# JeffreyXiang/ivid

Measured on NVIDIA H100. Metric: 128x128 RGBD multiview samples/sec, higher is better.
Workload: dtype fp16 tensor-core operands, fp32 accumulate / residual stream / GroupNorm / softmax / sampler

## Files before the change

### include/ivid_b200.h

```cpp
#ifndef IVID_B200_H_
#define IVID_B200_H_

#include <stdint.h>

#ifdef __cplusplus
extern "C" {
#endif

#define IVID_OK 0
#define IVID_ERR_INVALID_ARGUMENT 1
#define IVID_ERR_NOT_IMPLEMENTED 2
#define IVID_ERR_CUDA 3
#define IVID_ERR_STATE 4

typedef struct ivid_unet ivid_unet_t;
typedef struct ivid_sampler ivid_sampler_t;

const char* ivid_last_error(void);
int ivid_version(void);
int ivid_device_info(int device, int* sm_count, int* cc_major, int* cc_minor);


int ivid_unet_create(const char* cfg_json, ivid_unet_t** out);
int ivid_unet_destroy(ivid_unet_t* h);

int ivid_unet_num_params(const ivid_unet_t* h, int* count);
int ivid_unet_param_info(const ivid_unet_t* h, int index, const char** name, int64_t shape[4], int* ndim,
                         int* is_buffer);
int ivid_unet_set_param(ivid_unet_t* h, const char* name, const float* host_data, const int64_t* shape, int ndim);
int ivid_unet_finalize(ivid_unet_t* h, int device);
int ivid_unet_set_precision(ivid_unet_t* h, int precision);
int ivid_fp8_e4m3_quantize(const float* in, uint8_t* out, uint64_t count);
int ivid_fp8_weight_exponent(const float* w, uint64_t count, int* e_out);
int ivid_unet_weight_arena(const ivid_unet_t* h, void** dev_ptr, uint64_t* bytes);

int ivid_unet_forward(ivid_unet_t* h, const float* x_dev, int Nx, const int64_t* t_dev, const int64_t* classes_dev,
                      float* eps_dev, int N, void* stream);

int ivid_conv_tile(int H, int W, int* tw, int* th, int* tn, int* fused_stats);

int ivid_unet_debug_tap(ivid_unet_t* h, int N, const char* layer, float* host_out, uint64_t capacity, int* C, int* H, int* W);

int ivid_unet_profile_begin(ivid_unet_t* h);
int ivid_unet_profile_end(ivid_unet_t* h, char* json_out, int capacity);

typedef struct {
  int kind;
  const float* y_dev;
  const float* mask_dev;
  const float* mask_rgb_dev;
  const float* noise_dev;
  uint64_t seed;
  uint32_t stream_id;
  int sr_scale;
} ivid_cond_t;
int ivid_unet_forward_cond(ivid_unet_t* h, const float* x_dev, int Nx, const ivid_cond_t* cond, const int64_t* t_dev,
                           const int64_t* classes_dev, float* eps_dev, int N, void* stream);

int ivid_unet_forward_hw(ivid_unet_t* h, const float* x_dev, int Nx, int H, int W, const ivid_cond_t* cond,
                         const int64_t* t_dev, const int64_t* classes_dev, float* eps_dev, int N, void* stream);

int ivid_unet_forward_reuse(ivid_unet_t* h, const float* x_dev, int Nx, int H, int W, const ivid_cond_t* cond,
                            const int64_t* t_dev, const int64_t* classes_dev, float* eps_dev, int N, int cache_branch,
                            void* stream);


int ivid_sampler_create(const double* betas, int timesteps, ivid_sampler_t** out);
int ivid_sampler_destroy(ivid_sampler_t* s);
int ivid_sampler_table(const ivid_sampler_t* s, int which, double* out, int count);

typedef struct {
  int kind;
  int use_cfg;
  float strength;
  int clip_denoised;
  float eta;
  const int64_t* classes_dev;
  ivid_cond_t cond;
  const float* replace_rgb_dev;
  const float* replace_rgb_mask_dev;
  double replace_rgb_weight;
  const float* replace_depth_dev;
  const float* replace_depth_mask_dev;
  double replace_depth_weight;
  const float* constrain_depth_dev;
  double constrain_depth_weight;
  const float* step_noise_dev;
  uint64_t seed;
  int height, width;
  int order;
  const float* prev_x0_dev;
  int t_last;
// ... 108 lines not shown
```

### ivid_b200/_lib.py

```python
from __future__ import annotations

import ctypes
import os
from ctypes import POINTER, Structure, byref, c_char_p, c_double, c_float, c_int, c_int64, c_uint32, c_uint64, c_void_p

_HERE = os.path.dirname(os.path.abspath(__file__))
LIB_PATH = os.path.join(_HERE, "libivid_b200.so")

IVID_OK = 0
IVID_ERR_INVALID_ARGUMENT = 1
IVID_ERR_NOT_IMPLEMENTED = 2
IVID_ERR_CUDA = 3
IVID_ERR_STATE = 4


class CondT(Structure):
    _fields_ = [
        ("kind", c_int),
        ("y_dev", c_void_p),
        ("mask_dev", c_void_p),
        ("mask_rgb_dev", c_void_p),
        ("noise_dev", c_void_p),
        ("seed", c_uint64),
        ("stream_id", c_uint32),
# ... 39 lines not shown


class OpConvT(Structure):
    _fields_ = [
        ("act0_dev", c_void_p), ("C0", c_int), ("ksize", c_int), ("w0_host", c_void_p), ("b0_host", c_void_p),
        ("e4m3", c_int), ("e_out", POINTER(c_int)),
        ("act1_dev", c_void_p), ("C1", c_int), ("act2_dev", c_void_p), ("C2", c_int), ("wskip_host", c_void_p),
        ("bskip_host", c_void_p),
        ("residual_dev", c_void_p), ("residual_up", c_int),
        ("N", c_int), ("H", c_int), ("W", c_int), ("Cout", c_int),
        ("out_dev", c_void_p), ("out_mode", c_int), ("out16_dev", c_void_p), ("stats_dev", c_void_p),
    ]


class OpGnT(Structure):
    _fields_ = [
        ("x0_dev", c_void_p), ("C0", c_int), ("x1_dev", c_void_p), ("C1", c_int), ("x_fp16", c_int),
        ("stats0_dev", c_void_p), ("stats1_dev", c_void_p),
        ("N", c_int), ("H", c_int), ("W", c_int), ("groups", c_int), ("eps", c_float),
        ("gamma_host", c_void_p), ("beta_host", c_void_p),
        ("film_dev", c_void_p), ("film_ld", c_int), ("film_off", c_int), ("film_add", c_int),
        ("silu", c_int), ("mode", c_int),
        ("out_dev", c_void_p), ("out_e4m3", c_int), ("out_lo_dev", c_void_p), ("out_raw16_dev", c_void_p),
        ("out_raw32_dev", c_void_p),
    ]


class WarpParamsT(Structure):
    _fields_ = [("fov_deg", c_double), ("near", c_double), ("far", c_double), ("atol", c_double), ("rtol", c_double),
                ("erode_rgb", c_int), ("padding", c_double)]


SIGNATURES = {
    "ivid_last_error": (c_char_p, []),
    "ivid_version": (c_int, []),
    "ivid_device_info": (c_int, [c_int, POINTER(c_int), POINTER(c_int), POINTER(c_int)]),
    "ivid_unet_create": (c_int, [c_char_p, POINTER(c_void_p)]),
    "ivid_unet_destroy": (c_int, [c_void_p]),
    "ivid_unet_num_params": (c_int, [c_void_p, POINTER(c_int)]),
    "ivid_unet_param_info": (c_int, [c_void_p, c_int, POINTER(c_char_p), POINTER(c_int64), POINTER(c_int), POINTER(c_int)]),
    "ivid_unet_set_param": (c_int, [c_void_p, c_char_p, c_void_p, POINTER(c_int64), c_int]),
    "ivid_unet_finalize": (c_int, [c_void_p, c_int]),
    "ivid_unet_weight_arena": (c_int, [c_void_p, POINTER(c_void_p), POINTER(c_uint64)]),
    "ivid_unet_set_precision": (c_int, [c_void_p, c_int]),
    "ivid_fp8_e4m3_quantize": (c_int, [c_void_p, c_void_p, c_uint64]),
    "ivid_fp8_weight_exponent": (c_int, [c_void_p, c_uint64, POINTER(c_int)]),
    "ivid_unet_forward": (c_int, [c_void_p, c_void_p, c_int, c_void_p, c_void_p, c_void_p, c_int, c_void_p]),
    "ivid_unet_forward_cond": (c_int, [c_void_p, c_void_p, c_int, POINTER(CondT), c_void_p, c_void_p, c_void_p, c_int, c_void_p]),
    "ivid_unet_forward_hw": (c_int, [c_void_p, c_void_p, c_int, c_int, c_int, POINTER(CondT), c_void_p, c_void_p, c_void_p, c_int,
                                     c_void_p]),
    "ivid_unet_forward_reuse": (c_int, [c_void_p, c_void_p, c_int, c_int, c_int, POINTER(CondT), c_void_p, c_void_p, c_void_p,
                                        c_int, c_int, c_void_p]),
    "ivid_conv_tile": (c_int, [c_int, c_int, POINTER(c_int), POINTER(c_int), POINTER(c_int), POINTER(c_int)]),
    "ivid_unet_debug_tap": (c_int, [c_void_p, c_int, c_char_p, c_void_p, c_uint64, POINTER(c_int), POINTER(c_int), POINTER(c_int)]),
    "ivid_unet_profile_begin": (c_int, [c_void_p]),
    "ivid_unet_profile_end": (c_int, [c_void_p, c_char_p, c_int]),
    "ivid_sampler_create": (c_int, [POINTER(c_double), c_int, POINTER(c_void_p)]),
    "ivid_sampler_destroy": (c_int, [c_void_p]),
    "ivid_sampler_table": (c_int, [c_void_p, c_int, POINTER(c_double), c_int]),
    "ivid_sampler_step": (c_int, [c_void_p, c_void_p, c_void_p, c_void_p, c_void_p, c_int, c_int, c_int, POINTER(StepArgsT), c_void_p]),
    "ivid_sampler_step_dev": (c_int, [c_void_p, c_void_p, c_void_p, c_void_p, c_void_p, c_int, c_void_p, c_void_p, POINTER(StepArgsT), c_void_p]),
    "ivid_cfg_mix": (c_int, [c_void_p, c_float, c_void_p, c_uint64, c_void_p]),
    "ivid_op_dynamic_threshold": (c_int, [c_void_p, c_int, c_int, c_double, c_double, c_void_p, c_void_p, c_void_p]),
    "ivid_sampler_run": (c_int, [c_void_p, c_void_p, c_void_p, c_int, c_int, POINTER(StepArgsT), c_void_p, c_void_p, c_void_p, c_void_p, c_void_p]),
    "ivid_op_conv2d": (c_int, [c_void_p, c_int, c_int, c_int, c_int, c_void_p, c_void_p, c_int, c_int, c_void_p, c_int,
                               c_void_p, c_void_p, c_void_p, c_void_p, c_int, c_void_p]),
    "ivid_op_group_norm": (c_int, [c_void_p, c_int, c_void_p, c_int, c_int, c_int, c_int, c_int, c_float, c_void_p, c_void_p,
                                   c_void_p, c_int, c_int, c_void_p, c_void_p]),
    "ivid_op_conv2d_e4m3": (c_int, [c_void_p, c_int, c_int, c_int, c_int, c_void_p, c_void_p, c_int, c_int, c_void_p, c_int,
                                    c_void_p, c_void_p, c_void_p, c_void_p, c_int, POINTER(c_int), c_void_p]),
    "ivid_op_group_norm_e4m3": (c_int, [c_void_p, c_int, c_void_p, c_int, c_int, c_int, c_int, c_int, c_float, c_void_p,
                                        c_void_p, c_void_p, c_int, c_int, c_void_p, c_void_p]),
    "ivid_op_conv2d_ex": (c_int, [POINTER(OpConvT), c_void_p]),
    "ivid_op_group_norm_apply": (c_int, [POINTER(OpGnT), c_void_p]),
    "ivid_op_attention": (c_int, [c_void_p, c_int, c_int, c_int, c_void_p, c_void_p]),
    "ivid_op_attention_heads": (c_int, [c_void_p, c_int, c_int, c_int, c_int, c_void_p, c_void_p]),
    "ivid_warp_create": (c_int, [c_int, c_int, c_int, c_int, c_double, c_double, c_int, POINTER(c_void_p)]),
    "ivid_warp_destroy": (c_int, [c_void_p]),
    "ivid_warp_reset": (c_int, [c_void_p]),
    "ivid_warp_num_views": (c_int, [c_void_p, POINTER(c_int)]),
    "ivid_warp_add_view": (c_int, [c_void_p, c_void_p, c_void_p, c_int, POINTER(WarpParamsT), c_void_p]),
    "ivid_warp_mesh_from_depth": (c_int, [c_void_p, c_void_p, c_void_p, POINTER(WarpParamsT), c_void_p, c_void_p, c_void_p]),
    "ivid_warp_set_mesh": (c_int, [c_void_p, c_int, c_int, c_void_p, c_void_p, c_void_p, c_void_p]),
    "ivid_warp_get_mesh": (c_int, [c_void_p, c_int, c_int, c_void_p, c_void_p, c_void_p]),
    "ivid_warp_render": (c_int, [c_void_p, c_void_p, c_int, c_double, c_void_p, c_void_p, c_void_p, c_void_p, c_void_p]),
    "ivid_warp_aggregate": (c_int, [c_void_p, c_void_p, c_int, POINTER(WarpParamsT), c_void_p, c_void_p]),
    "ivid_warp_resolve_frame": (c_int, [c_void_p, c_double, c_double, c_void_p, c_void_p, c_void_p, c_void_p]),
    "ivid_warp_render_simple": (c_int, [c_void_p, c_void_p, c_int, c_void_p, c_int, c_void_p, c_void_p, c_double, c_void_p, c_void_p, c_void_p, c_void_p]),
    "ivid_warp_forward_backward": (c_int, [c_void_p, c_void_p, c_void_p, c_void_p, c_void_p, c_int, POINTER(WarpParamsT), c_void_p, c_void_p]),
    "ivid_warp_postfilter": (c_int, [c_void_p, c_void_p, c_void_p, c_void_p, c_void_p, POINTER(WarpParamsT), c_void_p, c_void_p]),
}

_lib = None


def lib() -> ctypes.CDLL:
    global _lib
    if _lib is None:
        if not os.path.exists(LIB_PATH):
            raise ImportError(
                f"{LIB_PATH} not found: build it with `python -m ivid_b200.build` (ivid_b200 has no CPU fallback)")
        l = ctypes.CDLL(LIB_PATH)
        for name, (res, args) in SIGNATURES.items():
            try:
                fn = getattr(l, name)
            except AttributeError:
# ... 33 lines not shown
```

### ivid_b200/csrc/api.cu

```cuda
#include <algorithm>
#include <cmath>
#include <cstring>
#include <memory>
#include <string>
#include <vector>

#include "../../include/ivid_b200.h"
#include "ops.h"
#include "sampler.h"
#include "unet.h"

using namespace ivid;

struct ivid_unet { std::unique_ptr<Unet> impl; };
struct ivid_sampler { std::unique_ptr<Sampler> impl; };

static thread_local std::string g_last_error;
namespace ivid { void set_last_error(const std::string& msg) { g_last_error = msg; } }

template <class F>
static int guarded(F&& f) {
  try {
    f();
    return IVID_OK;
// ... 84 lines not shown
  return guarded([&] {
    IVID_REQUIRE(count == 0 || w != nullptr, "w must not be NULL");
    IVID_NOT_NULL(e_out);
    float mx = 0.f;
    for (uint64_t i = 0; i < count; ++i) mx = std::max(mx, std::fabs(w[i]));
    *e_out = fp8_weight_exponent(mx);
  });
}
int ivid_unet_weight_arena(const ivid_unet_t* h, void** dev_ptr, uint64_t* bytes) {
  return guarded([&] {
    IVID_NOT_NULL(h);
    if (!h->impl->finalized()) throw Error(kErrState, "weight arena requested before finalize");
    if (dev_ptr) *dev_ptr = h->impl->arena();
    if (bytes) *bytes = h->impl->arena_bytes();
  });
}
int ivid_unet_forward_hw(ivid_unet_t* h, const float* x_dev, int Nx, int H, int W, const ivid_cond_t* cond,
                         const int64_t* t_dev, const int64_t* classes_dev, float* eps_dev, int N, void* stream) {
  return guarded([&] {
    IVID_NOT_NULL(h); IVID_NOT_NULL(x_dev); IVID_NOT_NULL(t_dev); IVID_NOT_NULL(eps_dev);
    h->impl->forward(x_dev, Nx, H, W, cond, t_dev, classes_dev, eps_dev, N, static_cast<cudaStream_t>(stream));
  });
}
int ivid_unet_forward_reuse(ivid_unet_t* h, const float* x_dev, int Nx, int H, int W, const ivid_cond_t* cond,
                            const int64_t* t_dev, const int64_t* classes_dev, float* eps_dev, int N, int cache_branch,
                            void* stream) {
  return guarded([&] {
    IVID_NOT_NULL(h); IVID_NOT_NULL(x_dev); IVID_NOT_NULL(t_dev); IVID_NOT_NULL(eps_dev);
    IVID_REQUIRE(cache_branch >= 0, "cache_branch must be in [0, num_res_blocks]");
    h->impl->forward(x_dev, Nx, H, W, cond, t_dev, classes_dev, eps_dev, N, static_cast<cudaStream_t>(stream), nullptr,
                     cache_branch);
  });
}
int ivid_unet_forward(ivid_unet_t* h, const float* x_dev, int Nx, const int64_t* t_dev, const int64_t* classes_dev,
                      float* eps_dev, int N, void* stream) {
  const int S = h != nullptr ? h->impl->cfg().image_size : 0;
  return ivid_unet_forward_hw(h, x_dev, Nx, S, S, nullptr, t_dev, classes_dev, eps_dev, N, stream);
}
int ivid_unet_forward_cond(ivid_unet_t* h, const float* x_dev, int Nx, const ivid_cond_t* cond, const int64_t* t_dev,
                           const int64_t* classes_dev, float* eps_dev, int N, void* stream) {
  if (cond == nullptr) return guarded([&] { IVID_NOT_NULL(cond); });
  const int S = h != nullptr ? h->impl->cfg().image_size : 0;
  return ivid_unet_forward_hw(h, x_dev, Nx, S, S, cond, t_dev, classes_dev, eps_dev, N, stream);
}

int ivid_conv_tile(int H, int W, int* tw, int* th, int* tn, int* fused_stats) {
  return guarded([&] {
    int a, b, c;
    conv_tile(H, W, &a, &b, &c);
    if (tw) *tw = a;
    if (th) *th = b;
    if (tn) *tn = c;
    if (fused_stats) *fused_stats = conv_can_fuse_stats(H, W) ? 1 : 0;
  });
}

int ivid_unet_debug_tap(ivid_unet_t* h, int N, const char* layer, float* host_out, uint64_t capacity, int* C, int* H, int* W) {
  return guarded([&] {
    IVID_NOT_NULL(h); IVID_NOT_NULL(layer);
    h->impl->debug_tap(N, layer, host_out, static_cast<size_t>(capacity), C, H, W);
  });
}

int ivid_unet_profile_begin(ivid_unet_t* h) {
  return guarded([&] { IVID_NOT_NULL(h); h->impl->profile_begin(); });
}
int ivid_unet_profile_end(ivid_unet_t* h, char* json_out, int capacity) {
  return guarded([&] {
    IVID_NOT_NULL(h); IVID_NOT_NULL(json_out);
    const std::string js = h->impl->profile_end();
    IVID_REQUIRE(static_cast<int>(js.size()) < capacity, "profile buffer too small");
    std::memcpy(json_out, js.c_str(), js.size() + 1);
  });
}

int ivid_sampler_create(const double* betas, int timesteps, ivid_sampler_t** out) {
  return guarded([&] {
    IVID_NOT_NULL(betas); IVID_NOT_NULL(out);
    auto s = std::make_unique<ivid_sampler>();
    s->impl = std::make_unique<Sampler>(betas, timesteps);
    *out = s.release();
  });
}
int ivid_sampler_destroy(ivid_sampler_t* s) {
  return guarded([&] { delete s; });
}
int ivid_sampler_table(const ivid_sampler_t* s, int which, double* out, int count) {
  return guarded([&] {
    IVID_NOT_NULL(s); IVID_NOT_NULL(out);
    const auto& t = s->impl->table(which);
    IVID_REQUIRE(count == static_cast<int>(t.size()), "table length mismatch");
    std::memcpy(out, t.data(), sizeof(double) * t.size());
  });
}
int ivid_sampler_step(ivid_sampler_t* s, ivid_unet_t* unet, const float* x_t_dev, float* x_prev_dev, float* pred_x0_dev,
                      int N, int t, int t_prev, const ivid_step_args_t* args, void* stream) {
  return guarded([&] {
    IVID_NOT_NULL(s); IVID_NOT_NULL(unet); IVID_NOT_NULL(x_t_dev); IVID_NOT_NULL(x_prev_dev); IVID_NOT_NULL(args);
    s->impl->step(*unet->impl, x_t_dev, x_prev_dev, pred_x0_dev, N, t, t_prev, *args, t, static_cast<cudaStream_t>(stream));
  });
}
int ivid_sampler_step_dev(ivid_sampler_t* s, ivid_unet_t* unet, const float* x_t_dev, float* x_prev_dev, float* pred_x0_dev,
                          int N, const int64_t* t_dev, const int64_t* t_prev_dev, const ivid_step_args_t* args, void* stream) {
  return guarded([&] {
    IVID_NOT_NULL(s); IVID_NOT_NULL(unet); IVID_NOT_NULL(x_t_dev); IVID_NOT_NULL(x_prev_dev); IVID_NOT_NULL(args); IVID_NOT_NULL(t_dev);
    IVID_REQUIRE(args->kind == 0 || t_prev_dev != nullptr, "DDIM / DPM-Solver++ step needs t_prev");
// ... 179 lines not shown
```

### ivid_b200/csrc/conv_gemm.cuh

```cuda
#pragma once
#include <type_traits>

#include "common.cuh"

namespace ivid {

struct ConvGemmParams {
  int N, H, W;
  int TW, TH, TN;
  int tiles_w, tiles_h, tiles_n;
  int n_blocks;
  int seg_chunks[3];
  int seg_taps[3];
  int Cout;
  int ldc;
  int ldr;
  int out_mode;
  const float* bias;
  const float* residual;
  int res_up;
  void* out;
  __half* out16;
  double* stats;
  float acc_scale;
};

struct ConvMaps {
  CUtensorMap a[3];
  CUtensorMap b;
};
struct ConvMaps8 : ConvMaps {
  CUtensorMap b8;
};

template <int BN, bool SLAB = false>
struct ConvGemmCfg {
  static constexpr int BM = 128;
  static constexpr int BK = 64;
  static constexpr int A_BYTES = BM * BK * 2;
  static constexpr int B_BYTES = ((BN * BK * 2 + 1023) / 1024) * 1024;
  static constexpr int STAGE_BYTES = A_BYTES + B_BYTES;
  static constexpr int STAGES = BN == 128 && !SLAB ? 3 : 4;
  static constexpr int SLAB_BYTES = 16 * 10 * 128;
  static constexpr int SLAB_STAGES = 2;
  static constexpr int RING_BYTES = SLAB ? SLAB_STAGES * SLAB_BYTES + STAGES * B_BYTES : STAGES * STAGE_BYTES;
  static constexpr int BAR_BYTES = 128;
  static constexpr int STAT_BYTES = 8 * 2 * BN * 4;
  static constexpr bool STATS_ON_RING = SLAB;
  static constexpr int SMEM_BYTES = RING_BYTES + BAR_BYTES + (STATS_ON_RING ? 0 : STAT_BYTES) + 1024;
  static constexpr int CONSUMER_THREADS = 256;
  static constexpr int THREADS = CONSUMER_THREADS + 32;
};

struct ConvKCursor {
  int seg = 0, t = 0, ch = 0, base = 0;
};

template <int BN, bool A8 = false, bool SLAB = false>
__global__ void __launch_bounds__(ConvGemmCfg<BN>::THREADS, 2)
conv_gemm_kernel(const __grid_constant__ std::conditional_t<A8, ConvMaps8, ConvMaps> maps, const __grid_constant__ ConvGemmParams p) {
  using Cfg = ConvGemmCfg<BN, SLAB>;
  constexpr int STAGES = Cfg::STAGES;
  constexpr int SLAB_STAGES = Cfg::SLAB_STAGES;
  extern __shared__ uint8_t smem_raw[];
  uint8_t* smem = smem_raw + ((1024u - (smem_u32(smem_raw) & 1023u)) & 1023u);
  uint64_t* full_bar = reinterpret_cast<uint64_t*>(smem + Cfg::RING_BYTES);
  uint64_t* empty_bar = full_bar + STAGES;
  uint64_t* slab_full = empty_bar + STAGES;
  uint64_t* slab_empty = slab_full + SLAB_STAGES;
  float* stat_smem = reinterpret_cast<float*>(Cfg::STATS_ON_RING ? smem : smem + Cfg::RING_BYTES + Cfg::BAR_BYTES);
  uint8_t* const slab_ring = smem;
  uint8_t* const w_ring = smem + SLAB_STAGES * Cfg::SLAB_BYTES;

  const int tid = threadIdx.x;
  const int warp = tid >> 5, lane = tid & 31;
  const int wg = warp >> 2;

  if (tid == 0) {
    for (int s = 0; s < STAGES; ++s) {
      mbar_init(&full_bar[s], 1);
      mbar_init(&empty_bar[s], 8u);
    }
    if constexpr (SLAB) {
      for (int s = 0; s < SLAB_STAGES; ++s) {
        mbar_init(&slab_full[s], 1);
        mbar_init(&slab_empty[s], 8u);
      }
    }
    fence_barrier_init();
  }
  __syncthreads();

  int nunits = 0;
  for (int sg = 0; sg < 3; ++sg) nunits += p.seg_chunks[sg] * p.seg_taps[sg];
  const int nunits8 = A8 ? p.seg_chunks[0] * p.seg_taps[0] : 0;

  const int mt = static_cast<int>(blockIdx.x) / p.n_blocks, nb = static_cast<int>(blockIdx.x) % p.n_blocks;
  const int colbase = nb * BN;
  const int tiles_per_img = p.tiles_w * p.tiles_h;
  const int tn = mt / tiles_per_img;
  const int rem = mt - tn * tiles_per_img;
  const int th = rem / p.tiles_w;
  const int tw = rem - th * p.tiles_w;
  const int n0 = tn * p.TN, h0 = th * p.TH, w0 = tw * p.TW;

  if (warp == Cfg::CONSUMER_THREADS / 32) {
    if (lane == 0) {
      tma_prefetch_desc(&maps.a[0]);
      tma_prefetch_desc(&maps.b);
      if constexpr (A8) tma_prefetch_desc(&maps.b8);
      if constexpr (SLAB) {
        const uint32_t slab_bytes = static_cast<uint32_t>(p.TW * (p.TH + 2)) * 128u;
        uint32_t u = 0, a = 0;
        int base = 0;
#pragma unroll 1
        for (int sg = 0; sg < 3; ++sg) {
          const int chunks = p.seg_chunks[sg];
          const int nx = p.seg_taps[sg] == 9 ? 3 : 1;
          const bool e4m3 = A8 && sg == 0;
#pragma unroll 1
          for (int ch = 0; ch < chunks; ++ch) {
#pragma unroll 1
            for (int xi = 0; xi < nx; ++xi, ++a) {
              const int sl = static_cast<int>(a % SLAB_STAGES);
              if (a >= SLAB_STAGES) mbar_wait(&slab_empty[sl], ((a / SLAB_STAGES) - 1) & 1);
              mbar_arrive_expect_tx(&slab_full[sl], nx == 3 ? slab_bytes : static_cast<uint32_t>(Cfg::A_BYTES));
              tma_load_4d(&maps.a[sg], &slab_full[sl], slab_ring + sl * Cfg::SLAB_BYTES, ch * (e4m3 ? 128 : 64),
                          w0 + (nx == 3 ? xi - 1 : 0), h0 - (nx == 3 ? 1 : 0), n0);
#pragma unroll 1
              for (int yi = 0; yi < nx; ++yi, ++u) {
                const int s = static_cast<int>(u % STAGES);
                if (u >= STAGES) mbar_wait(&empty_bar[s], ((u / STAGES) - 1) & 1);
                mbar_arrive_expect_tx(&full_bar[s], BN * Cfg::BK * 2);
                const int t = nx == 3 ? 3 * yi + xi : 0;
                uint8_t* sb = w_ring + s * Cfg::B_BYTES;
                if constexpr (A8) {
                  if (e4m3) { tma_load_2d(&maps.b8, &full_bar[s], sb, (t * chunks + ch) * 128, colbase); continue; }
                }
                tma_load_2d(&maps.b, &full_bar[s], sb, base + (t * chunks + ch) * 64, colbase);
// ... 133 lines not shown
    const int c = colbase + 8 * j + 2 * quad;
    float s0 = 0.f, s1 = 0.f, q0 = 0.f, q1 = 0.f;
    if (c < p.Cout) {
      const float2 b = make_float2(__ldg(p.bias + c), __ldg(p.bias + c + 1));
#pragma unroll
      for (int i = 0; i < 2; ++i) {
        if (!ok[i]) continue;
        float v0, v1;
        if (A8) {
          v0 = fmaf(acc[4 * j + 2 * i], p.acc_scale, b.x); v1 = fmaf(acc[4 * j + 2 * i + 1], p.acc_scale, b.y);
        } else {
          v0 = acc[4 * j + 2 * i] + b.x; v1 = acc[4 * j + 2 * i + 1] + b.y;
        }
        if (p.out_mode == 2) {
          const uint32_t hw = static_cast<uint32_t>(p.H) * p.W, n = pix[i] / hw;
          float* o = reinterpret_cast<float*>(p.out) + (static_cast<size_t>(n) * p.Cout + c) * hw + (pix[i] - n * hw);
          o[0] = v0;
          if (c + 1 < p.Cout) o[hw] = v1;
          continue;
        }
        if (p.residual != nullptr) {
          const float2 r = __ldg(reinterpret_cast<const float2*>(p.residual + static_cast<size_t>(rpix[i]) * p.ldr + c));
          v0 += r.x; v1 += r.y;
        }
        if (p.out_mode == 0) {
          *reinterpret_cast<float2*>(reinterpret_cast<float*>(p.out) + static_cast<size_t>(pix[i]) * p.ldc + c) = make_float2(v0, v1);
          if (p.out16 != nullptr) *reinterpret_cast<uint32_t*>(p.out16 + static_cast<size_t>(pix[i]) * p.ldc + c) = pack_h2(v0, v1);
        } else {
          const __half2 hv = __floats2half2_rn(v0, v1);
          *reinterpret_cast<__half2*>(reinterpret_cast<__half*>(p.out) + static_cast<size_t>(pix[i]) * p.ldc + c) = hv;
          const float2 r = __half22float2(hv);
          v0 = r.x; v1 = r.y;
        }
        s0 += v0; s1 += v1;
        q0 = fmaf(v0, v0, q0); q1 = fmaf(v1, v1, q1);
      }
    }
    if (do_stats) {
#pragma unroll
      for (int off = 4; off < 32; off <<= 1) {
        s0 += __shfl_xor_sync(0xffffffffu, s0, off);
        s1 += __shfl_xor_sync(0xffffffffu, s1, off);
        q0 += __shfl_xor_sync(0xffffffffu, q0, off);
        q1 += __shfl_xor_sync(0xffffffffu, q1, off);
      }
      if (lane < 4) {
        float* st = stat_smem + warp * 2 * BN + 8 * j + 2 * quad;
        st[0] = s0; st[1] = s1; st[BN] = q0; st[BN + 1] = q1;
      }
    }
  }
  if (do_stats) {
    asm volatile("bar.sync 1, %0;\n" ::"n"(Cfg::CONSUMER_THREADS) : "memory");
    const int rows_per_n = p.TW * p.TH;
    const int n_tile = (128 + rows_per_n - 1) / rows_per_n;
    for (int e = tid; e < n_tile * BN; e += Cfg::CONSUMER_THREADS) {
      const int sn = e / BN, c = e - sn * BN;
      const int n = n0 + sn, col = colbase + c;
      if (n >= p.N || col >= p.Cout) continue;
      float ssum = 0.f, qsum = 0.f;
      for (int w8 = 0; w8 < 8; ++w8) {
        if ((w8 * 16) / rows_per_n != sn) continue;
        ssum += stat_smem[w8 * 2 * BN + c];
        qsum += stat_smem[w8 * 2 * BN + BN + c];
      }
      double* st = p.stats + (static_cast<size_t>(n) * p.Cout + col) * 2;
      atomicAdd(st, static_cast<double>(ssum));
      atomicAdd(st + 1, static_cast<double>(qsum));
    }
  }
}

}
```

### ivid_b200/csrc/ops.cu

```cuda
#include "ops.h"

#include <algorithm>
#include <cmath>
#include <mutex>

#include "attention.cuh"
#include "attention_hd.cuh"
#include "conv_gemm.cuh"
#include "elementwise.cuh"
#include "embed.cuh"

namespace ivid {

struct ConvLaunch {
  ConvMaps8 maps;
  ConvGemmParams p;
  int BN;
  bool a8;
  bool slab;
  int grid;
};

int conv_pad_cout(int cout) {
  if (cout >= 64) return ((cout + 63) / 64) * 64;
  return ((cout + 15) / 16) * 16;
}
static int pow2_divisor(int v, int cap) {
  int t = 1;
  while (t * 2 <= cap && v % (t * 2) == 0) t *= 2;
  return t;
}
void conv_tile(int H, int W, int* TW, int* TH, int* TN) {
  IVID_REQUIRE(H > 0 && W > 0, "conv: spatial size must be positive");
  *TW = pow2_divisor(W, 16);
  *TH = pow2_divisor(H, 128 / *TW);
  *TN = 128 / (*TW * *TH);
}
bool conv_can_fuse_stats(int H, int W) {
  int TW, TH, TN;
  conv_tile(H, W, &TW, &TH, &TN);
  return TW * TH >= 32;
}
int conv_pick_bn(int cout_pad) {
  if (cout_pad % 128 == 0) return 128;
  if (cout_pad % 64 == 0) return 64;
  if (cout_pad % 16 == 0 && cout_pad <= 48) return 16;
  throw Error(kErrInvalidArgument, "conv: unsupported padded Cout " + std::to_string(cout_pad));
}

bool conv_can_res_up(int W, int cout) { return W >= 16 && cout % 8 == 0; }
bool conv_can_out16(int cout) { return cout % 8 == 0; }
int conv_pad_k(int c) { return ((c + 63) / 64) * 64; }
int conv_pad_k8(int c) { return ((c + 127) / 128) * 128; }
int conv_seg_cols(int taps, int c) { return taps * conv_pad_k(c); }

ConvPack conv_pack(const float* w, const float* b, int cout, int cin, int ksz, int pitch, const float* w2, const float* b2,
                   int cin2, int cin2a, bool e4m3) {
  ConvPack pk;
  const int taps = ksz * ksz;
  pk.cout_pad = conv_pad_cout(cout);
  float scale = 1.f;
  if (e4m3) {
    IVID_REQUIRE(pitch == conv_pad_k(cin), "internal: an e4m3 segment 0 is an ordinary 3x3 or 1x1 conv");
    float mx = 0.f;
    for (size_t i = 0; i < static_cast<size_t>(cout) * cin * taps; ++i) mx = std::max(mx, std::fabs(w[i]));
    const int e = fp8_weight_exponent(mx);
    const float kMinNormal16 = std::ldexp(1.0f, -14);
    if (cin % 16 != 0) pk.refused = "its input channels are not a multiple of 16";
    else if (e < -100 || e > 100) pk.refused = "its weight exponent is outside [-100, 100]";
    for (size_t i = 0; pk.refused == nullptr && i < static_cast<size_t>(cout) * cin2; ++i) {
      const float v = std::fabs(w2[i]), sv = v * std::ldexp(1.0f, e);
      if (sv > 65504.f) pk.refused = "its skip weights times 2^e overflow fp16";
      else if (v >= kMinNormal16 && sv < kMinNormal16) pk.refused = "its skip weights times 2^e become fp16 subnormals";
    }
    pk.e4m3 = pk.refused == nullptr;
    if (pk.e4m3) { pk.e = e; scale = std::ldexp(1.0f, e); }
  }
  const int s0 = cin2a > 0 ? cin2a : cin2, s1 = cin2 - s0;
  const int k0 = pk.e4m3 ? 0 : conv_seg_cols(1, taps * pitch);
  pk.K = k0 + conv_seg_cols(1, s0) + conv_seg_cols(1, s1);
  pk.w16.assign(static_cast<size_t>(pk.cout_pad) * pk.K, __float2half_rn(0.f));
  const int cp8 = conv_pad_k8(cin), K8 = pk.e4m3 ? taps * cp8 : 0;
  pk.w8.assign(static_cast<size_t>(pk.cout_pad) * K8, 0);
  for (int co = 0; co < cout; ++co) {
    __half* row = pk.w16.data() + static_cast<size_t>(co) * pk.K;
    for (int tap = 0; tap < taps; ++tap)
      for (int ci = 0; ci < cin; ++ci) {
        const float v = w[(static_cast<size_t>(co) * cin + ci) * taps + tap];
        if (pk.e4m3) pk.w8[static_cast<size_t>(co) * K8 + tap * cp8 + ci] = fp8_e4m3_from_float(v * scale);
        else row[tap * pitch + ci] = __float2half_rn(v);
      }
    for (int ci = 0; ci < cin2; ++ci)
      row[k0 + (ci < s0 ? ci : conv_pad_k(s0) + ci - s0)] = __float2half_rn(w2[static_cast<size_t>(co) * cin2 + ci] * scale);
  }
  pk.bias.assign(pk.cout_pad, 0.f);
  for (int i = 0; i < cout; ++i) {
    if (b != nullptr) pk.bias[i] = b[i];
    if (b2 != nullptr) pk.bias[i] += b2[i];
  }
  return pk;
}

ConvLaunch* conv_launch_create(const ConvDesc& d) {
  IVID_REQUIRE(d.C0 > 0 && d.C0 % 8 == 0, "conv: segment-0 channels must be a positive multiple of 8");
  IVID_REQUIRE(d.C1 % 8 == 0, "conv: segment-1 channels must be a multiple of 8");
  IVID_REQUIRE(d.taps0 == 9 || d.taps0 == 1, "conv: only 3x3 (pad 1) and 1x1 kernels are on this path");
  IVID_REQUIRE(d.taps1 == 9 || d.taps1 == 1, "conv: only 3x3 (pad 1) and 1x1 kernels are on this path");
  IVID_REQUIRE(d.C2 % 8 == 0 && (d.taps2 == 9 || d.taps2 == 1), "conv: segment 2 must be a multiple of 8 channels, 3x3 or 1x1");
  IVID_REQUIRE(d.N > 0 && static_cast<int64_t>(d.N) * d.H * d.W < (int64_t{1} << 31),
               "conv: N*H*W must be below 2^31 (32-bit pixel indices in the epilogue)");
  const bool a8 = d.weight8 != nullptr;
  IVID_REQUIRE(!a8 || d.C0 % 16 == 0, "conv: an e4m3 segment 0 needs a multiple of 16 channels (16-byte TMA rows)");
  auto* l = new ConvLaunch();
  l->a8 = a8;
  ConvGemmParams& p = l->p;
  p.N = d.N; p.H = d.H; p.W = d.W;
  conv_tile(d.H, d.W, &p.TW, &p.TH, &p.TN);
  p.tiles_w = d.W / p.TW;
  p.tiles_h = d.H / p.TH;
  p.tiles_n = (d.N + p.TN - 1) / p.TN;
  const bool any3x3 = d.taps0 == 9 || (d.C1 > 0 && d.taps1 == 9) || (d.C2 > 0 && d.taps2 == 9);
  l->slab = any3x3 && p.TN == 1 && p.TW >= 8;
  IVID_REQUIRE(!l->slab || p.TW * (p.TH + 2) * 128 <= (ConvGemmCfg<128, true>::SLAB_BYTES), "internal: conv slab larger than its slot");
  l->BN = conv_pick_bn(d.cout_pad);
  p.n_blocks = d.cout_pad / l->BN;
  p.seg_chunks[0] = a8 ? conv_pad_k8(d.C0) / 128 : conv_pad_k(d.C0) / 64; p.seg_taps[0] = d.taps0;
  p.acc_scale = d.acc_scale;
  p.seg_chunks[1] = conv_pad_k(d.C1) / 64; p.seg_taps[1] = d.C1 > 0 ? d.taps1 : 0;
  p.seg_chunks[2] = conv_pad_k(d.C2) / 64; p.seg_taps[2] = d.C2 > 0 ? d.taps2 : 0;
  p.Cout = d.cout; p.ldc = d.ldc; p.ldr = d.ldr; p.out_mode = d.out_mode;
  p.bias = d.bias; p.residual = d.residual; p.out = d.out;
  p.stats = (d.stats != nullptr && conv_can_fuse_stats(d.H, d.W) && d.out_mode != 2) ? d.stats : nullptr;
  IVID_REQUIRE(d.stats == nullptr || p.stats != nullptr, "conv: fused statistics need >= 32 pixels per sample per warp");
  IVID_REQUIRE(d.out_mode == 2 || (d.cout % 8 == 0 && d.ldc % 8 == 0), "conv: NHWC output needs Cout % 8 == 0");
  IVID_REQUIRE(d.residual == nullptr || (d.out_mode != 2 && d.ldr % 2 == 0), "conv: residual needs an NHWC output and an even row pitch");
  p.res_up = 0;
  if (d.residual != nullptr && d.residual_up) {
    IVID_REQUIRE(conv_can_res_up(d.W, d.cout) && d.H % 2 == 0, "conv: upsampled residual needs W >= 16 and Cout % 8 == 0");
    p.res_up = 1;
  }
  p.out16 = nullptr;
  if (d.out16 != nullptr) {
    IVID_REQUIRE(d.out_mode == 0 && conv_can_out16(d.cout), "conv: fp16 output copy needs an fp32 NHWC output and Cout % 8 == 0");
    p.out16 = static_cast<__half*>(d.out16);
  }
  const int Ktot = (a8 ? 0 : conv_seg_cols(d.taps0, d.C0)) + conv_seg_cols(d.taps1, d.C1) + conv_seg_cols(d.taps2, d.C2);
  ConvMaps8& M = l->maps;
  auto rows = [&](int taps) { return l->slab && taps == 9 ? p.TH + 2 : p.TH; };
  M.a[0] = a8 ? make_act_map(d.act0, d.N, d.H, d.W, d.C0, p.TW, rows(d.taps0), p.TN, CU_TENSOR_MAP_DATA_TYPE_UINT8)
              : make_act_map(d.act0, d.N, d.H, d.W, d.C0, p.TW, rows(d.taps0), p.TN);
  M.a[1] = d.C1 > 0 ? make_act_map(d.act1, d.N, d.H, d.W, d.C1, p.TW, rows(d.taps1), p.TN) : M.a[0];
  M.a[2] = d.C2 > 0 ? make_act_map(d.act2, d.N, d.H, d.W, d.C2, p.TW, rows(d.taps2), p.TN) : M.a[0];
  if (a8) {
    M.b8 = make_weight_map(d.weight8, d.cout_pad, d.taps0 * conv_pad_k8(d.C0), l->BN, CU_TENSOR_MAP_DATA_TYPE_UINT8);
    M.b = Ktot > 0 ? make_weight_map(d.weight, d.cout_pad, Ktot, l->BN) : M.b8;
  } else {
    M.b = make_weight_map(d.weight, d.cout_pad, Ktot, l->BN);
  }
  l->grid = p.tiles_w * p.tiles_h * p.tiles_n * p.n_blocks;
  return l;
}
void conv_launch_destroy(ConvLaunch* l) { delete l; }
int conv_launch_bn(const ConvLaunch* l) { return l->BN; }
bool conv_launch_a8(const ConvLaunch* l) { return l->a8; }

template <int BN, bool A8, bool SLAB>
static void run_conv(const ConvLaunch* l, cudaStream_t s) {
  using Cfg = ConvGemmCfg<BN, SLAB>;
  static std::once_flag once;
  std::call_once(once, [] {
    IVID_CHECK_CUDA(cudaFuncSetAttribute(conv_gemm_kernel<BN, A8, SLAB>, cudaFuncAttributeMaxDynamicSharedMemorySize, Cfg::SMEM_BYTES));
  });
  if constexpr (A8) conv_gemm_kernel<BN, true, SLAB><<<l->grid, Cfg::THREADS, Cfg::SMEM_BYTES, s>>>(l->maps, l->p);
  else conv_gemm_kernel<BN, false, SLAB><<<l->grid, Cfg::THREADS, Cfg::SMEM_BYTES, s>>>(static_cast<const ConvMaps&>(l->maps), l->p);
  IVID_CHECK_CUDA(cudaGetLastError());
}
template <bool A8, bool SLAB>
static void run_conv_bn(const ConvLaunch* l, cudaStream_t s) {
  switch (l->BN) {
    case 128: run_conv<128, A8, SLAB>(l, s); break;
    case 64: run_conv<64, A8, SLAB>(l, s); break;
    default: run_conv<16, A8, SLAB>(l, s); break;
  }
}
void conv_launch_run_out(const ConvLaunch* l, void* out, cudaStream_t s) {
  ConvLaunch tmp = *l;
  tmp.p.out = out;
  conv_launch_run(&tmp, s);
}
void conv_launch_run(const ConvLaunch* l, cudaStream_t s) {
  if (l->a8) {
    if (l->slab) run_conv_bn<true, true>(l, s);
    else run_conv_bn<true, false>(l, s);
  } else {
    if (l->slab) run_conv_bn<false, true>(l, s);
    else run_conv_bn<false, false>(l, s);
  }
}

struct AttnLaunch {
  CUtensorMap mapQ, mapKV;
  AttnParams p;
  AttnHdParams hp;
  int head_ch = 64;
  int nv = 0;
  bool qres = false;
  int smem = 0;
  int grid;
};

AttnLaunch* attn_launch_create(const void* qkv, int N, int T, int C, int head_ch, void* out) {
  if (head_ch <= 0 || head_ch % 64 != 0)
    throw Error(kErrNotImplemented, "attention: head width " + std::to_string(head_ch) + " is not a multiple of 64");
  IVID_REQUIRE(C % head_ch == 0, "attention: channels must be a multiple of the head width " + std::to_string(head_ch));
  IVID_REQUIRE(T >= 1, "attention: sequence length must be positive");
  auto* l = new AttnLaunch();
  l->head_ch = head_ch;
  l->p.N = N; l->p.T = T; l->p.C = C; l->p.heads = C / 64;
  l->p.q_tiles = (T + 127) / 128;
  l->p.out = reinterpret_cast<__half*>(out);
  const uint64_t dims[3] = {static_cast<uint64_t>(3 * C), static_cast<uint64_t>(T), static_cast<uint64_t>(N)};
  const uint64_t str[2] = {static_cast<uint64_t>(3 * C) * 2, static_cast<uint64_t>(T) * 3 * C * 2};
  const uint32_t boxq[3] = {64, 128, 1};
  const uint32_t boxkv[3] = {64, AttnCfg::KV, 1};
  l->mapQ = make_tensor_map(CU_TENSOR_MAP_DATA_TYPE_FLOAT16, 3, const_cast<void*>(qkv), dims, str, boxq,
                            CU_TENSOR_MAP_SWIZZLE_128B);
  l->mapKV = make_tensor_map(CU_TENSOR_MAP_DATA_TYPE_FLOAT16, 3, const_cast<void*>(qkv), dims, str, boxkv,
                             CU_TENSOR_MAP_SWIZZLE_128B);
  l->grid = N * l->p.heads * l->p.q_tiles;
  if (head_ch == 64) return l;
  using Cfg = AttnHdCfg;
  const int k = head_ch / 64;
  const int slices = (k + 3) / 4;
  l->nv = (k + slices - 1) / slices;
  l->qres = k <= Cfg::RESIDENT_Q_MAX_CHUNKS;
  AttnHdParams& hp = l->hp;
  hp.N = N; hp.T = T; hp.C = C; hp.d = head_ch; hp.heads = C / head_ch; hp.chunks = k;
  hp.q_tiles = l->p.q_tiles;
  hp.slices = (k + l->nv - 1) / l->nv;
  hp.scale_log2 = static_cast<float>(1.4426950408889634 / std::sqrt(static_cast<double>(head_ch)));
  hp.out = l->p.out;
  const int q_bytes = l->qres ? k * Cfg::QCHUNK_BYTES : 0;
  const int fixed = q_bytes + 1024  + 1024 ;
// ... 189 lines not shown
```

### ivid_b200/csrc/ops.h

```cpp
#pragma once
#include <cuda.h>
#include <cuda_fp16.h>
#include <cuda_runtime.h>
#include <stdint.h>

#include <vector>

#include "host_util.h"

namespace ivid {

struct ConvLaunch;
struct AttnLaunch;

struct ConvDesc {
  const void* act0 = nullptr; int C0 = 0; int taps0 = 9;
  const void* act1 = nullptr; int C1 = 0; int taps1 = 1;
  const void* act2 = nullptr; int C2 = 0; int taps2 = 1;
  void* out16 = nullptr;
  const void* weight = nullptr;
  const void* weight8 = nullptr;
  float acc_scale = 1.f;
  int cout_pad = 0;
  int cout = 0;
  const float* bias = nullptr;
  const float* residual = nullptr; int ldr = 0;
  bool residual_up = false;
  void* out = nullptr; int ldc = 0; int out_mode = 0;
  double* stats = nullptr;
  int N = 0, H = 0, W = 0;
};

ConvLaunch* conv_launch_create(const ConvDesc& d);
void conv_launch_destroy(ConvLaunch* l);
void conv_launch_run(const ConvLaunch* l, cudaStream_t s);
int conv_launch_bn(const ConvLaunch* l);
bool conv_launch_a8(const ConvLaunch* l);
void conv_launch_run_out(const ConvLaunch* l, void* out, cudaStream_t s);
int conv_pick_bn(int cout_pad);
bool conv_can_out16(int cout);
bool conv_can_res_up(int W, int cout);
void conv_tile(int H, int W, int* TW, int* TH, int* TN);
bool conv_can_fuse_stats(int H, int W);
int conv_pad_cout(int cout);
int conv_pad_k(int c);
int conv_pad_k8(int c);
int conv_seg_cols(int taps, int c);

struct ConvPack {
  std::vector<__half> w16;
  std::vector<uint8_t> w8;
  std::vector<float> bias;
  int cout_pad = 0, K = 0;
  bool e4m3 = false;
  int e = 0;
  const char* refused = nullptr;
};
ConvPack conv_pack(const float* w, const float* b, int cout, int cin, int ksz, int pitch, const float* w2, const float* b2,
                   int cin2, int cin2a, bool e4m3);

AttnLaunch* attn_launch_create(const void* qkv, int N, int T, int C, int head_ch, void* out);
void attn_launch_destroy(AttnLaunch* l);
void attn_launch_run(const AttnLaunch* l, cudaStream_t s);

void launch_gn_stats(const float* x, double* stats, int N, int HW, int C, cudaStream_t s);
struct GnApplyDesc {
  const void* x0 = nullptr; const void* x1 = nullptr; int C0 = 0, C1 = 0;
  bool x0_half = false;
  int N = 0, H = 0, W = 0; int mode = 0; int silu = 1;
  const double* stats0 = nullptr; const double* stats1 = nullptr;
  int groups = 32; float eps = 1e-5f;
  const float* gamma = nullptr; const float* beta = nullptr;
  const float* film = nullptr; int film_ld = 0, film_off = 0;
  bool film_add = false;
  void* out_act = nullptr; void* out_raw16 = nullptr; float* out_raw32 = nullptr;
  void* out_lo = nullptr;
  bool out_e4m3 = false;
};
void launch_gn_apply(const GnApplyDesc& d, cudaStream_t s);
void launch_eps_gather(const float* Y, const float* bias, float* eps, int N, int H, int W, int Co, int ldy, cudaStream_t s);
void launch_im2col_s2(const void* x16, void* col, int N, int H, int W, int C, cudaStream_t s);
void launch_upsample2x_h16(const void* x16, void* out, int N, int H, int W, int C, cudaStream_t s);
void launch_resample_f32(const float* x, float* out, void* out16, int N, int H, int W, int C, int mode, cudaStream_t s);
void launch_pack_input(const float* x, void* out, int N, int Nx, int Cin, int HW, cudaStream_t s);

struct CondPackDesc {
  const float* x = nullptr; const float* y = nullptr; const float* mask = nullptr; const float* mask_rgb = nullptr;
  const float* noise = nullptr; void* out = nullptr; int N = 0, Nx = 0, H = 0, W = 0; int kind = 0;
  int scale = 2;
  uint64_t seed = 0; uint32_t stream = 0; const int* stream_dev = nullptr;
};
void launch_cond_pack(const CondPackDesc& d, cudaStream_t s);
void launch_cfg_mix(const float* eps2, float* out, size_t count, float strength, cudaStream_t s);
void launch_dynamic_threshold(const float* x, int N, int M, double ratio, double threshold_max, float* s_out, float* x_out,
                              cudaStream_t s);
// ... 8 lines not shown
```

Baseline: 0.3264.

## Add 256-pixel M tile for lone 3x3 slab convolutions on large grids

Adds a BM=256 variant of the warp-specialized conv GEMM kernel that doubles the consumer warps and covers a 16x16 spatial slab per CTA. It is used only for plain 3x3 convs with BN=128 when enough CTAs exist to fill the SMs several times over. The larger tile is meant to let each B (weight) tile and each slab halo be reused across more output pixels, cutting load traffic per output. The cost is one block per SM instead of two, larger shared memory use, and a separate GroupNorm-statistics reduction path written for this tile shape.

```diff
diff --git a/include/ivid_b200.h b/include/ivid_b200.h
--- a/include/ivid_b200.h
+++ b/include/ivid_b200.h
@@ -38,6 +38,9 @@
                       float* eps_dev, int N, void* stream);
 
 int ivid_conv_tile(int H, int W, int* tw, int* th, int* tn, int* fused_stats);
+
+int ivid_conv_tile_class(int N, int H, int W, int cout, int ksize, int skip_channels, int residual, int* tw, int* th,
+                         int* tn, int* bm);
 
 int ivid_unet_debug_tap(ivid_unet_t* h, int N, const char* layer, float* host_out, uint64_t capacity, int* C, int* H, int* W);
 
diff --git a/ivid_b200/_lib.py b/ivid_b200/_lib.py
--- a/ivid_b200/_lib.py
+++ b/ivid_b200/_lib.py
@@ -115,6 +115,8 @@
     "ivid_unet_forward_reuse": (c_int, [c_void_p, c_void_p, c_int, c_int, c_int, POINTER(CondT), c_void_p, c_void_p, c_void_p,
                                         c_int, c_int, c_void_p]),
     "ivid_conv_tile": (c_int, [c_int, c_int, POINTER(c_int), POINTER(c_int), POINTER(c_int), POINTER(c_int)]),
+    "ivid_conv_tile_class": (c_int, [c_int, c_int, c_int, c_int, c_int, c_int, c_int, POINTER(c_int), POINTER(c_int),
+                                     POINTER(c_int), POINTER(c_int)]),
     "ivid_unet_debug_tap": (c_int, [c_void_p, c_int, c_char_p, c_void_p, c_uint64, POINTER(c_int), POINTER(c_int), POINTER(c_int)]),
     "ivid_unet_profile_begin": (c_int, [c_void_p]),
     "ivid_unet_profile_end": (c_int, [c_void_p, c_char_p, c_int]),
diff --git a/ivid_b200/csrc/api.cu b/ivid_b200/csrc/api.cu
--- a/ivid_b200/csrc/api.cu
+++ b/ivid_b200/csrc/api.cu
@@ -160,6 +160,22 @@
     if (th) *th = b;
     if (tn) *tn = c;
     if (fused_stats) *fused_stats = conv_can_fuse_stats(H, W) ? 1 : 0;
+  });
+}
+
+int ivid_conv_tile_class(int N, int H, int W, int cout, int ksize, int skip_channels, int residual, int* tw, int* th, int* tn,
+                         int* bm) {
+  return guarded([&] {
+    IVID_REQUIRE(N > 0 && cout > 0 && (ksize == 3 || ksize == 1) && skip_channels >= 0,
+                 "conv tile class: N, Cout > 0, a 3x3 or 1x1 kernel and skip channels >= 0");
+    int a, b, c;
+    conv_tile(H, W, &a, &b, &c);
+    const int m = conv_pick_bm(N, H, W, conv_pad_cout(cout), ksize == 3 && skip_channels == 0 && residual == 0);
+    if (m == 256) b = 16;
+    if (tw) *tw = a;
+    if (th) *th = b;
+    if (tn) *tn = c;
+    if (bm) *bm = m;
   });
 }
 
diff --git a/ivid_b200/csrc/conv_gemm.cuh b/ivid_b200/csrc/conv_gemm.cuh
--- a/ivid_b200/csrc/conv_gemm.cuh
+++ b/ivid_b200/csrc/conv_gemm.cuh
@@ -33,33 +33,36 @@
   CUtensorMap b8;
 };
 
-template <int BN, bool SLAB = false>
+template <int BN, bool SLAB = false, int TILE_M = 128>
 struct ConvGemmCfg {
-  static constexpr int BM = 128;
+  static constexpr int BM = TILE_M;
   static constexpr int BK = 64;
   static constexpr int A_BYTES = BM * BK * 2;
   static constexpr int B_BYTES = ((BN * BK * 2 + 1023) / 1024) * 1024;
   static constexpr int STAGE_BYTES = A_BYTES + B_BYTES;
   static constexpr int STAGES = BN == 128 && !SLAB ? 3 : 4;
-  static constexpr int SLAB_BYTES = 16 * 10 * 128;
+  static constexpr int SLAB_BYTES = 16 * (BM / 16 + 2) * 128;
   static constexpr int SLAB_STAGES = 2;
   static constexpr int RING_BYTES = SLAB ? SLAB_STAGES * SLAB_BYTES + STAGES * B_BYTES : STAGES * STAGE_BYTES;
   static constexpr int BAR_BYTES = 128;
-  static constexpr int STAT_BYTES = 8 * 2 * BN * 4;
+  static constexpr int STAT_BYTES = (BM / 16) * 2 * BN * 4;
   static constexpr bool STATS_ON_RING = SLAB;
   static constexpr int SMEM_BYTES = RING_BYTES + BAR_BYTES + (STATS_ON_RING ? 0 : STAT_BYTES) + 1024;
-  static constexpr int CONSUMER_THREADS = 256;
+  static constexpr int CONSUMER_THREADS = 2 * BM;
   static constexpr int THREADS = CONSUMER_THREADS + 32;
+  static constexpr int MIN_BLOCKS = BM == 128 ? 2 : 1;
+  static_assert(BM == 128 || (BM == 256 && SLAB && BN == 128), "the 256-pixel tile is a BN 128 slab tile");
 };
 
 struct ConvKCursor {
   int seg = 0, t = 0, ch = 0, base = 0;
 };
 
-template <int BN, bool A8 = false, bool SLAB = false>
-__global__ void __launch_bounds__(ConvGemmCfg<BN>::THREADS, 2)
+template <int BN, bool A8 = false, bool SLAB = false, int BM = 128>
+__global__ void __launch_bounds__(ConvGemmCfg<BN, SLAB, BM>::THREADS, ConvGemmCfg<BN, SLAB, BM>::MIN_BLOCKS)
 conv_gemm_kernel(const __grid_constant__ std::conditional_t<A8, ConvMaps8, ConvMaps> maps, const __grid_constant__ ConvGemmParams p) {
-  using Cfg = ConvGemmCfg<BN, SLAB>;
+  using Cfg = ConvGemmCfg<BN, SLAB, BM>;
+  constexpr uint32_t CONSUMER_WARPS = Cfg::CONSUMER_THREADS / 32;
   constexpr int STAGES = Cfg::STAGES;
   constexpr int SLAB_STAGES = Cfg::SLAB_STAGES;
   extern __shared__ uint8_t smem_raw[];
@@ -79,12 +82,12 @@
   if (tid == 0) {
     for (int s = 0; s < STAGES; ++s) {
       mbar_init(&full_bar[s], 1);
-      mbar_init(&empty_bar[s], 8u);
+      mbar_init(&empty_bar[s], CONSUMER_WARPS);
     }
     if constexpr (SLAB) {
       for (int s = 0; s < SLAB_STAGES; ++s) {
         mbar_init(&slab_full[s], 1);
-        mbar_init(&slab_empty[s], 8u);
+        mbar_init(&slab_empty[s], CONSUMER_WARPS);
       }
     }
     fence_barrier_init();
@@ -324,21 +327,37 @@
   }
   if (do_stats) {
     asm volatile("bar.sync 1, %0;\n" ::"n"(Cfg::CONSUMER_THREADS) : "memory");
-    const int rows_per_n = p.TW * p.TH;
-    const int n_tile = (128 + rows_per_n - 1) / rows_per_n;
-    for (int e = tid; e < n_tile * BN; e += Cfg::CONSUMER_THREADS) {
-      const int sn = e / BN, c = e - sn * BN;
-      const int n = n0 + sn, col = colbase + c;
-      if (n >= p.N || col >= p.Cout) continue;
-      float ssum = 0.f, qsum = 0.f;
-      for (int w8 = 0; w8 < 8; ++w8) {
-        if ((w8 * 16) / rows_per_n != sn) continue;
-        ssum += stat_smem[w8 * 2 * BN + c];
-        qsum += stat_smem[w8 * 2 * BN + BN + c];
-      }
-      double* st = p.stats + (static_cast<size_t>(n) * p.Cout + col) * 2;
-      atomicAdd(st, static_cast<double>(ssum));
-      atomicAdd(st + 1, static_cast<double>(qsum));
+    if constexpr (BM == 256) {
+      for (int e = tid; e < 2 * BN; e += Cfg::CONSUMER_THREADS) {
+        const int hf = e / BN, c = e - hf * BN;
+        const int col = colbase + c;
+        if (col >= p.Cout) continue;
+        float ssum = 0.f, qsum = 0.f;
+        for (int w8 = 0; w8 < 8; ++w8) {
+          ssum += stat_smem[(8 * hf + w8) * 2 * BN + c];
+          qsum += stat_smem[(8 * hf + w8) * 2 * BN + BN + c];
+        }
+        double* st = p.stats + (static_cast<size_t>(n0) * p.Cout + col) * 2;
+        atomicAdd(st, static_cast<double>(ssum));
+        atomicAdd(st + 1, static_cast<double>(qsum));
+      }
+    } else {
+      const int rows_per_n = p.TW * p.TH;
+      const int n_tile = (128 + rows_per_n - 1) / rows_per_n;
+      for (int e = tid; e < n_tile * BN; e += Cfg::CONSUMER_THREADS) {
+        const int sn = e / BN, c = e - sn * BN;
+        const int n = n0 + sn, col = colbase + c;
+        if (n >= p.N || col >= p.Cout) continue;
+        float ssum = 0.f, qsum = 0.f;
+        for (int w8 = 0; w8 < 8; ++w8) {
+          if ((w8 * 16) / rows_per_n != sn) continue;
+          ssum += stat_smem[w8 * 2 * BN + c];
+          qsum += stat_smem[w8 * 2 * BN + BN + c];
+        }
+        double* st = p.stats + (static_cast<size_t>(n) * p.Cout + col) * 2;
+        atomicAdd(st, static_cast<double>(ssum));
+        atomicAdd(st + 1, static_cast<double>(qsum));
+      }
     }
   }
 }
diff --git a/ivid_b200/csrc/ops.cu b/ivid_b200/csrc/ops.cu
--- a/ivid_b200/csrc/ops.cu
+++ b/ivid_b200/csrc/ops.cu
@@ -18,6 +18,7 @@
   int BN;
   bool a8;
   bool slab;
+  int bm;
   int grid;
 };
 
@@ -35,6 +36,13 @@
   *TW = pow2_divisor(W, 16);
   *TH = pow2_divisor(H, 128 / *TW);
   *TN = 128 / (*TW * *TH);
+}
+int conv_pick_bm(int N, int H, int W, int cout_pad, bool lone3x3) {
+  int TW, TH, TN;
+  conv_tile(H, W, &TW, &TH, &TN);
+  if (!lone3x3 || TN != 1 || TW != 16 || H % 16 != 0 || conv_pick_bn(cout_pad) != 128) return 128;
+  const int64_t ctas = static_cast<int64_t>(N) * (H / 16) * (W / 16) * (cout_pad / 128);
+  return ctas >= 3 * static_cast<int64_t>(sm_count()) ? 256 : 128;
 }
 bool conv_can_fuse_stats(int H, int W) {
   int TW, TH, TN;
@@ -121,8 +129,14 @@
   p.tiles_n = (d.N + p.TN - 1) / p.TN;
   const bool any3x3 = d.taps0 == 9 || (d.C1 > 0 && d.taps1 == 9) || (d.C2 > 0 && d.taps2 == 9);
   l->slab = any3x3 && p.TN == 1 && p.TW >= 8;
-  IVID_REQUIRE(!l->slab || p.TW * (p.TH + 2) * 128 <= (ConvGemmCfg<128, true>::SLAB_BYTES), "internal: conv slab larger than its slot");
   l->BN = conv_pick_bn(d.cout_pad);
+  l->bm = conv_pick_bm(d.N, d.H, d.W, d.cout_pad, d.taps0 == 9 && d.C1 == 0 && d.C2 == 0 && d.residual == nullptr);
+  if (l->bm == 256) {
+    p.TH = 16;
+    p.tiles_h = d.H / p.TH;
+  }
+  IVID_REQUIRE(!l->slab || p.TW * (p.TH + 2) * 128 <= (l->bm == 256 ? ConvGemmCfg<128, true, 256>::SLAB_BYTES : ConvGemmCfg<128, true>::SLAB_BYTES),
+               "internal: conv slab larger than its slot");
   p.n_blocks = d.cout_pad / l->BN;
   p.seg_chunks[0] = a8 ? conv_pad_k8(d.C0) / 128 : conv_pad_k(d.C0) / 64; p.seg_taps[0] = d.taps0;
   p.acc_scale = d.acc_scale;
@@ -164,15 +178,15 @@
 int conv_launch_bn(const ConvLaunch* l) { return l->BN; }
 bool conv_launch_a8(const ConvLaunch* l) { return l->a8; }
 
-template <int BN, bool A8, bool SLAB>
+template <int BN, bool A8, bool SLAB, int BM = 128>
 static void run_conv(const ConvLaunch* l, cudaStream_t s) {
-  using Cfg = ConvGemmCfg<BN, SLAB>;
+  using Cfg = ConvGemmCfg<BN, SLAB, BM>;
   static std::once_flag once;
   std::call_once(once, [] {
-    IVID_CHECK_CUDA(cudaFuncSetAttribute(conv_gemm_kernel<BN, A8, SLAB>, cudaFuncAttributeMaxDynamicSharedMemorySize, Cfg::SMEM_BYTES));
+    IVID_CHECK_CUDA(cudaFuncSetAttribute(conv_gemm_kernel<BN, A8, SLAB, BM>, cudaFuncAttributeMaxDynamicSharedMemorySize, Cfg::SMEM_BYTES));
   });
-  if constexpr (A8) conv_gemm_kernel<BN, true, SLAB><<<l->grid, Cfg::THREADS, Cfg::SMEM_BYTES, s>>>(l->maps, l->p);
-  else conv_gemm_kernel<BN, false, SLAB><<<l->grid, Cfg::THREADS, Cfg::SMEM_BYTES, s>>>(static_cast<const ConvMaps&>(l->maps), l->p);
+  if constexpr (A8) conv_gemm_kernel<BN, true, SLAB, BM><<<l->grid, Cfg::THREADS, Cfg::SMEM_BYTES, s>>>(l->maps, l->p);
+  else conv_gemm_kernel<BN, false, SLAB, BM><<<l->grid, Cfg::THREADS, Cfg::SMEM_BYTES, s>>>(static_cast<const ConvMaps&>(l->maps), l->p);
   IVID_CHECK_CUDA(cudaGetLastError());
 }
 template <bool A8, bool SLAB>
@@ -189,6 +203,11 @@
   conv_launch_run(&tmp, s);
 }
 void conv_launch_run(const ConvLaunch* l, cudaStream_t s) {
+  if (l->bm == 256) {
+    if (l->a8) run_conv<128, true, true, 256>(l, s);
+    else run_conv<128, false, true, 256>(l, s);
+    return;
+  }
   if (l->a8) {
     if (l->slab) run_conv_bn<true, true>(l, s);
     else run_conv_bn<true, false>(l, s);
diff --git a/ivid_b200/csrc/ops.h b/ivid_b200/csrc/ops.h
--- a/ivid_b200/csrc/ops.h
+++ b/ivid_b200/csrc/ops.h
@@ -41,6 +41,7 @@
 bool conv_can_out16(int cout);
 bool conv_can_res_up(int W, int cout);
 void conv_tile(int H, int W, int* TW, int* TH, int* TN);
+int conv_pick_bm(int N, int H, int W, int cout_pad, bool lone3x3);
 bool conv_can_fuse_stats(int H, int W);
 int conv_pad_cout(int cout);
 int conv_pad_k(int c);
```

Result: faster. 0.3313, median of 6 (+1.5%).
